# riusricardo/midnight-bls12-381-cuda

Measured on AMD Instinct MI355X. Metric: G1 MSM/sec at 2^20 points + Fr NTT/sec at 2^22 (bit-exact vs BLST), higher is better.
Workload: dtype u32-limb Montgomery (Fq 381-bit / Fr 255-bit integer); 1 GPU; G1 MSM 2^20 points per GPU, production path (ICICLE entry, Montgomery scalars + bases in HBM, (x,y,1) result on device); N>1: sharded, RCCL all-gather of partial sums; msm_points_per_gpu=1048576, ntt_size=4194304, parallelism=msm-shard1

## Files before the change

include/bls12_381_mi355x.h:

```cpp
#ifndef BLS12_381_MI355X_H
#define BLS12_381_MI355X_H

#include <stddef.h>
#include <stdint.h>
#include <stdbool.h>

#ifdef __cplusplus
extern "C" {
#endif

typedef enum {
    MBLS_SUCCESS = 0,
    MBLS_INVALID_DEVICE = 1,
    MBLS_OUT_OF_MEMORY = 2,
    MBLS_INVALID_POINTER = 3,
    MBLS_ALLOCATION_FAILED = 4,
    MBLS_DEALLOCATION_FAILED = 5,
    MBLS_COPY_FAILED = 6,
    MBLS_SYNCHRONIZATION_FAILED = 7,
    MBLS_STREAM_CREATION_FAILED = 8,
    MBLS_STREAM_DESTRUCTION_FAILED = 9,
    MBLS_API_NOT_IMPLEMENTED = 10,
    MBLS_INVALID_ARGUMENT = 11,
    MBLS_BACKEND_LOAD_FAILED = 12,
// ... 176 lines not shown
eIcicleError bls12_381_g1_scalar_mul_glv(const mbls_g1_affine_t* bases, const mbls_fr_t* scalars, int size,
                                         const VecOpsConfig* config, mbls_g1_projective_t* output);
eIcicleError bls12_381_g2_scalar_mul(const mbls_g2_affine_t* bases, const mbls_fr_t* scalars, int size,
                                     const VecOpsConfig* config, mbls_g2_projective_t* output);
eIcicleError mbls_g1_scalar_mul(const mbls_g1_affine_t* bases, const mbls_fr_t* scalars, int size,
                                bool scalars_montgomery, const VecOpsConfig* config, mbls_g1_projective_t* output);
eIcicleError mbls_g2_scalar_mul(const mbls_g2_affine_t* bases, const mbls_fr_t* scalars, int size,
                                bool scalars_montgomery, const VecOpsConfig* config, mbls_g2_projective_t* output);

eIcicleError mbls_g1_ecntt(const mbls_g1_affine_t* input, int size, NTTDir dir, const NTTConfig* config,
                           mbls_g1_affine_t* output);

typedef enum {
    MBLS_POINT_OK = 0,
    MBLS_POINT_IDENTITY = 1,
    MBLS_POINT_NONCANONICAL = 2,
    MBLS_POINT_OFF_CURVE = 3,
    MBLS_POINT_OFF_SUBGROUP = 4
} mbls_point_status;

eIcicleError mbls_g1_check_points(const mbls_g1_affine_t* points, int size, bool points_montgomery,
                                  const VecOpsConfig* config, uint8_t* status, uint64_t* n_invalid);
eIcicleError mbls_g2_check_points(const mbls_g2_affine_t* points, int size, bool points_montgomery,
                                  const VecOpsConfig* config, uint8_t* status, uint64_t* n_invalid);

typedef enum {
    MBLS_DECODE_OK = 0,
    MBLS_DECODE_IDENTITY = 1,
    MBLS_DECODE_NONCANONICAL = 2,
    MBLS_DECODE_NO_POINT = 3,
    MBLS_DECODE_BAD_FLAGS = 5
} mbls_decode_status;

eIcicleError mbls_g1_decompress(const uint8_t* bytes, int size, bool points_montgomery, const VecOpsConfig* config,
                                mbls_g1_affine_t* points, uint8_t* status, uint64_t* n_invalid);
eIcicleError mbls_g2_decompress(const uint8_t* bytes, int size, bool points_montgomery, const VecOpsConfig* config,
                                mbls_g2_affine_t* points, uint8_t* status, uint64_t* n_invalid);
eIcicleError mbls_g1_compress(const mbls_g1_affine_t* points, int size, bool points_montgomery,
                              const VecOpsConfig* config, uint8_t* bytes);
eIcicleError mbls_g2_compress(const mbls_g2_affine_t* points, int size, bool points_montgomery,
                              const VecOpsConfig* config, uint8_t* bytes);

const char* mbls_version(void);
const char* mbls_error_string(eIcicleError e);
eIcicleError mbls_gen_scalars(mbls_fr_t* out_device, uint64_t seed, size_t n, bool montgomery, void* stream);
eIcicleError mbls_gen_g1_bases(mbls_g1_affine_t* out_device, uint64_t seed, size_t n, void* stream);
eIcicleError mbls_gen_g2_bases(mbls_g2_affine_t* out_device, uint64_t seed, size_t n, void* stream);
eIcicleError mbls_gen_scalars_range(mbls_fr_t* out_device, uint64_t seed, size_t start, size_t n, bool montgomery,
                                    void* stream);
eIcicleError mbls_gen_g1_bases_range(mbls_g1_affine_t* out_device, uint64_t seed, size_t start, size_t n, void* stream);
eIcicleError mbls_gen_g2_bases_range(mbls_g2_affine_t* out_device, uint64_t seed, size_t start, size_t n, void* stream);
eIcicleError mbls_g1_msm_jacobian(const mbls_fr_t* scalars, const mbls_g1_affine_t* bases, int msm_size,
                                  const MSMConfig* config, mbls_g1_projective_t* results);
eIcicleError mbls_g2_msm_jacobian(const mbls_fr_t* scalars, const mbls_g2_affine_t* bases, int msm_size,
                                  const MSMConfig* config, mbls_g2_projective_t* results);
eIcicleError mbls_g1_sum_jacobian(const mbls_g1_projective_t* points_device, int count,
                                  mbls_g1_projective_t* result_device, void* stream);
eIcicleError mbls_g2_sum_jacobian(const mbls_g2_projective_t* points_device, int count,
                                  mbls_g2_projective_t* result_device, void* stream);
eIcicleError mbls_g1_jacobian_to_icicle(mbls_g1_projective_t* points_device, int count, void* stream);
eIcicleError mbls_g2_jacobian_to_icicle(mbls_g2_projective_t* points_device, int count, void* stream);

eIcicleError mbls_release_stream(void* stream);
eIcicleError mbls_release_scratch(void);
void mbls_scratch_stats(uint64_t* mallocs, uint64_t* frees, uint64_t* bytes, int* contexts);

eIcicleError mbls_g1_msm_multi_device(const mbls_fr_t* scalars, const mbls_g1_affine_t* const* bases_per_dev,
                                      const int* devs, int ndev, int msm_size, const MSMConfig* config,
                                      mbls_g1_projective_t* result);
eIcicleError mbls_g2_msm_multi_device(const mbls_fr_t* scalars, const mbls_g2_affine_t* const* bases_per_dev,
                                      const int* devs, int ndev, int msm_size, const MSMConfig* config,
                                      mbls_g2_projective_t* result);

eIcicleError bls12_381_vector_sum(const mbls_fr_t* a, size_t size, const VecOpsConfig* config, mbls_fr_t* output);

eIcicleError mbls_msm_plan(int group, int msm_size, const MSMConfig* config, int32_t* out);

eIcicleError mbls_msm_reduce_plan(int group, int msm_size, const MSMConfig* config, int32_t* out, int capacity,
                                  int32_t* count);

eIcicleError mbls_msm_front_probe(int group, const mbls_fr_t* scalars, const void* bases, int msm_size,
                                  const MSMConfig* config, int64_t* info, void* const* tables);

void mbls_profile_enable(int on);
void mbls_profile_reset(void);
int mbls_profile_read(const char** names, double* total_ms, long* counts, int max);

eIcicleError mbls_msm_accumulate_event(void* stream, void* event);
eIcicleError mbls_msm_accumulate_event_drop(void* event);

eIcicleError mbls_msm_precompute_strict(int on);

#ifdef __cplusplus
}
#endif
#endif
```

midnight-bls12-381-cuda_amd/bls12_381_amd.py:

```python
from __future__ import annotations

import ctypes
import os

import numpy as np

HERE = os.path.dirname(os.path.abspath(__file__))
LIB_PATH = os.environ.get("MBLS_LIB") or os.path.join(HERE, "lib", "libbls12_381_mi355x.so")

ERRORS = ["SUCCESS", "INVALID_DEVICE", "OUT_OF_MEMORY", "INVALID_POINTER", "ALLOCATION_FAILED",
          "DEALLOCATION_FAILED", "COPY_FAILED", "SYNCHRONIZATION_FAILED", "STREAM_CREATION_FAILED",
          "STREAM_DESTRUCTION_FAILED", "API_NOT_IMPLEMENTED", "INVALID_ARGUMENT", "BACKEND_LOAD_FAILED",
          "LICENSE_CHECK_ERROR", "UNKNOWN_ERROR"]
SUCCESS, INVALID_POINTER, API_NOT_IMPLEMENTED, INVALID_ARGUMENT = 0, 3, 10, 11


class IcicleError(RuntimeError):
    def __init__(self, code, what):
        name = ERRORS[code] if 0 <= code < len(ERRORS) else str(code)
        super().__init__(f"{what} failed: {name} ({code})")
        self.code = code


class MSMConfig(ctypes.Structure):
    _fields_ = [("stream", ctypes.c_void_p), ("precompute_factor", ctypes.c_int), ("c", ctypes.c_int),
                ("bitsize", ctypes.c_int), ("batch_size", ctypes.c_int),
                ("are_points_shared_in_batch", ctypes.c_bool), ("are_scalars_on_device", ctypes.c_bool),
                ("are_scalars_montgomery_form", ctypes.c_bool), ("are_points_on_device", ctypes.c_bool),
                ("are_points_montgomery_form", ctypes.c_bool), ("are_results_on_device", ctypes.c_bool),
                ("is_async", ctypes.c_bool), ("ext", ctypes.c_void_p)]


class FrC(ctypes.Structure):
    _fields_ = [("limbs", ctypes.c_uint64 * 4)]


class NTTConfig(ctypes.Structure):
    _fields_ = [("stream", ctypes.c_void_p), ("coset_gen", FrC), ("batch_size", ctypes.c_int),
                ("columns_batch", ctypes.c_bool), ("ordering", ctypes.c_int),
                ("are_inputs_on_device", ctypes.c_bool), ("are_outputs_on_device", ctypes.c_bool),
                ("is_async", ctypes.c_bool), ("ext", ctypes.c_void_p)]


class NTTInitDomainConfig(ctypes.Structure):
    _fields_ = [("stream", ctypes.c_void_p), ("is_async", ctypes.c_bool), ("ext", ctypes.c_void_p)]


class VecOpsConfig(ctypes.Structure):
    _fields_ = [("stream", ctypes.c_void_p), ("is_a_on_device", ctypes.c_bool), ("is_b_on_device", ctypes.c_bool),
                ("is_result_on_device", ctypes.c_bool), ("is_async", ctypes.c_bool), ("batch_size", ctypes.c_int),
                ("columns_batch", ctypes.c_bool), ("ext", ctypes.c_void_p)]


EXPORTED = [
    "mbls_default_msm_config", "mbls_default_ntt_config", "mbls_default_vec_ops_config",
    "bls12_381_g1_msm_cuda", "bls12_381_g2_msm_cuda", "bls12_381_icicle_g1_msm", "bls12_381_icicle_g2_msm",
    "bls12_381_icicle_g1_msm_precompute_bases", "bls12_381_icicle_g2_msm_precompute_bases",
    "bls12_381_ntt_init_domain_cuda", "bls12_381_ntt_release_domain_cuda", "bls12_381_ntt_cuda",
    "bls12_381_coset_ntt_cuda", "bls12_381_field_ntt_cuda", "bls12_381_field_ntt_init_domain_cuda",
    "bls12_381_field_ntt_release_domain_cuda", "bls12_381_ntt_get_rou_from_domain",
    "bls12_381_vector_add", "bls12_381_vector_sub", "bls12_381_vector_mul", "bls12_381_scalar_mul_vec",
    "bls12_381_scalar_add_vec", "vec_add_cuda", "vec_sub_cuda", "vec_mul_cuda", "scalar_mul_vec_cuda",
    "scalar_add_vec_cuda", "vec_sum_cuda", "bls12_381_batch_inv_cuda",
    "mbls_version", "mbls_error_string", "mbls_gen_scalars", "mbls_gen_g1_bases", "mbls_gen_g2_bases",
    "mbls_gen_scalars_range", "mbls_gen_g1_bases_range", "mbls_gen_g2_bases_range",
    "mbls_g1_msm_jacobian", "mbls_g2_msm_jacobian",
    "mbls_g1_sum_jacobian", "mbls_g2_sum_jacobian", "mbls_g1_jacobian_to_icicle", "mbls_g2_jacobian_to_icicle",
    "mbls_profile_enable", "mbls_profile_reset", "mbls_profile_read",
    "mbls_release_stream", "mbls_release_scratch", "mbls_scratch_stats",
    "mbls_g1_msm_multi_device", "mbls_g2_msm_multi_device", "bls12_381_vector_sum",
    "bls12_381_g1_affine_to_projective", "bls12_381_g1_projective_to_affine", "bls12_381_g2_projective_to_affine",
    "mbls_msm_plan", "mbls_msm_reduce_plan", "mbls_msm_front_probe", "mbls_msm_accumulate_event", "mbls_msm_accumulate_event_drop", "mbls_msm_precompute_strict",
    "bls12_381_g1_scalar_mul", "bls12_381_g1_scalar_mul_glv", "bls12_381_g2_scalar_mul",
    "mbls_g1_scalar_mul", "mbls_g2_scalar_mul", "mbls_g1_ecntt",
    "mbls_g1_check_points", "mbls_g2_check_points",
    "mbls_g1_decompress", "mbls_g2_decompress", "mbls_g1_compress", "mbls_g2_compress",
    "mbls_fr_prefix_product", "mbls_fr_poly_divide_linear", "mbls_fr_scan_geometry",
    "mbls_fr_eval_program", "mbls_fr_expr_check",
    "mbls_fr_sort", "mbls_fr_lookup_permute", "mbls_fr_sort_plan",
    "mbls_fr_coeff_to_extended", "mbls_fr_extended_to_coeff", "mbls_fr_domain_plan",
    "mbls_fr_lookup_multiplicities", "mbls_fr_prefix_sum", "mbls_fr_logup_sum",
]

_LIB = None


def lib():
    global _LIB
    if _LIB is not None:
        return _LIB
    if not os.path.exists(LIB_PATH):
        raise RuntimeError(f"HIP library not built: {LIB_PATH} (run __graft_entry__.build())")
    L = ctypes.CDLL(LIB_PATH)
    P, E = ctypes.c_void_p, ctypes.c_int
    sz, i32, u64, b = ctypes.c_size_t, ctypes.c_int, ctypes.c_uint64, ctypes.c_bool
    sig = {
        "bls12_381_g1_msm_cuda": [P, P, i32, P, P], "bls12_381_g2_msm_cuda": [P, P, i32, P, P],
        "bls12_381_icicle_g1_msm": [P, P, i32, P, P], "bls12_381_icicle_g2_msm": [P, P, i32, P, P],
        "bls12_381_icicle_g1_msm_precompute_bases": [P, i32, P, P],
        "bls12_381_icicle_g2_msm_precompute_bases": [P, i32, P, P],
        "bls12_381_ntt_init_domain_cuda": [P, P], "bls12_381_ntt_release_domain_cuda": [],
        "bls12_381_ntt_cuda": [P, i32, i32, P, P], "bls12_381_coset_ntt_cuda": [P, i32, i32, P, P, P],
        "bls12_381_field_ntt_cuda": [P, i32, i32, P, P], "bls12_381_field_ntt_init_domain_cuda": [P, P],
        "bls12_381_field_ntt_release_domain_cuda": [], "bls12_381_ntt_get_rou_from_domain": [u64, P],
        "bls12_381_vector_add": [P, P, sz, P, P], "bls12_381_vector_sub": [P, P, sz, P, P],
        "bls12_381_vector_mul": [P, P, sz, P, P], "bls12_381_scalar_mul_vec": [P, P, sz, P, P],
        "bls12_381_scalar_add_vec": [P, P, sz, P, P],
        "vec_add_cuda": [P, P, P, i32, P], "vec_sub_cuda": [P, P, P, i32, P], "vec_mul_cuda": [P, P, P, i32, P],
        "scalar_mul_vec_cuda": [P, P, P, i32, P], "scalar_add_vec_cuda": [P, P, P, i32, P],
        "vec_sum_cuda": [P, P, i32, P], "bls12_381_batch_inv_cuda": [P, P, i32, P],
        "mbls_gen_scalars": [P, u64, sz, b, P], "mbls_gen_g1_bases": [P, u64, sz, P],
        "mbls_gen_g2_bases": [P, u64, sz, P], "mbls_g1_sum_jacobian": [P, i32, P, P],
        "mbls_gen_scalars_range": [P, u64, sz, sz, b, P], "mbls_gen_g1_bases_range": [P, u64, sz, sz, P],
        "mbls_gen_g2_bases_range": [P, u64, sz, sz, P],
        "mbls_g1_msm_jacobian": [P, P, i32, P, P], "mbls_g2_msm_jacobian": [P, P, i32, P, P],
        "mbls_g2_sum_jacobian": [P, i32, P, P], "mbls_g1_jacobian_to_icicle": [P, i32, P],
        "mbls_g2_jacobian_to_icicle": [P, i32, P],
        "mbls_release_stream": [P], "mbls_release_scratch": [],
        "mbls_g1_msm_multi_device": [P, P, P, i32, i32, P, P], "mbls_g2_msm_multi_device": [P, P, P, i32, i32, P, P],
        "bls12_381_vector_sum": [P, sz, P, P],
        "bls12_381_g1_affine_to_projective": [P, i32, P, P], "bls12_381_g1_projective_to_affine": [P, i32, P, P],
        "bls12_381_g2_projective_to_affine": [P, i32, P, P],
        "mbls_msm_plan": [i32, i32, P, P], "mbls_msm_reduce_plan": [i32, i32, P, P, i32, P],
        "mbls_msm_front_probe": [i32, P, P, i32, P, P, P],
        "mbls_msm_accumulate_event": [P, P], "mbls_msm_accumulate_event_drop": [P],
        "mbls_msm_precompute_strict": [i32],
        "bls12_381_g1_scalar_mul": [P, P, i32, P, P], "bls12_381_g1_scalar_mul_glv": [P, P, i32, P, P],
        "bls12_381_g2_scalar_mul": [P, P, i32, P, P],
        "mbls_g1_scalar_mul": [P, P, i32, b, P, P], "mbls_g2_scalar_mul": [P, P, i32, b, P, P],
        "mbls_g1_ecntt": [P, i32, i32, P, P],
        "mbls_g1_check_points": [P, i32, b, P, P, P], "mbls_g2_check_points": [P, i32, b, P, P, P],
        "mbls_g1_decompress": [P, i32, b, P, P, P, P], "mbls_g2_decompress": [P, i32, b, P, P, P, P],
        "mbls_g1_compress": [P, i32, b, P, P], "mbls_g2_compress": [P, i32, b, P, P],
        "mbls_fr_prefix_product": [P, P, sz, P, b, P, P, P], "mbls_fr_poly_divide_linear": [P, sz, P, P, P, P],
        "mbls_fr_scan_geometry": [sz, P],
        "mbls_fr_eval_program": [P, i32, sz, sz, P, i32, P, i32, i32, P, P],
        "mbls_fr_expr_check": [P, i32, i32, i32, i32, P],
        "mbls_fr_sort": [P, sz, b, P, P, P], "mbls_fr_lookup_permute": [P, P, sz, b, P, P, P, P],
        "mbls_fr_sort_plan": [sz, i32, P],
        "mbls_fr_coeff_to_extended": [P, i32, i32, P, P, P],
        "mbls_fr_extended_to_coeff": [P, i32, i32, P, P, i32, P, P], "mbls_fr_domain_plan": [i32, i32, P],
        "mbls_fr_lookup_multiplicities": [P, i32, P, sz, b, b, P, P, P],
        "mbls_fr_prefix_sum": [P, sz, P, b, P, P, P], "mbls_fr_logup_sum": [P, i32, P, P, sz, P, P, P, P, P],
    }
    for name, args in sig.items():
        f = getattr(L, name)
        f.argtypes = args
        f.restype = E
    L.mbls_version.restype = ctypes.c_char_p
    L.mbls_error_string.restype = ctypes.c_char_p
    L.mbls_error_string.argtypes = [E]
    L.mbls_default_msm_config.restype = MSMConfig
    L.mbls_default_ntt_config.restype = NTTConfig
    L.mbls_default_vec_ops_config.restype = VecOpsConfig
    L.mbls_profile_enable.argtypes = [ctypes.c_int]
    L.mbls_profile_enable.restype = None
    L.mbls_profile_reset.argtypes = []
    L.mbls_profile_reset.restype = None
    L.mbls_profile_read.argtypes = [ctypes.POINTER(ctypes.c_char_p), ctypes.POINTER(ctypes.c_double),
                                    ctypes.POINTER(ctypes.c_long), ctypes.c_int]
    L.mbls_profile_read.restype = ctypes.c_int
    L.mbls_scratch_stats.argtypes = [ctypes.POINTER(ctypes.c_uint64)] * 3 + [ctypes.POINTER(ctypes.c_int)]
    L.mbls_scratch_stats.restype = None
    _LIB = L
    return L


def profile(enable=True):
    lib().mbls_profile_enable(1 if enable else 0)
    lib().mbls_profile_reset()


def profile_read():
    n = 64
    names = (ctypes.c_char_p * n)()
    ms = (ctypes.c_double * n)()
    cnt = (ctypes.c_long * n)()
    k = lib().mbls_profile_read(names, ms, cnt, n)
    return {names[i].decode(): (ms[i], cnt[i]) for i in range(min(k, n))}


def check(code, what):
    if code != SUCCESS:
        raise IcicleError(code, what)


def _p(x):
    if x is None:
        return None
    if isinstance(x, np.ndarray):
        assert x.flags["C_CONTIGUOUS"]
        return ctypes.c_void_p(x.ctypes.data)
    return ctypes.c_void_p(x.data_ptr())


def _is_dev(x):
    return x is not None and not isinstance(x, np.ndarray) and bool(getattr(x, "is_cuda", True))


def _stream_handle(stream):
    if stream is None:
        return None
    if isinstance(stream, int):
        return ctypes.c_void_p(stream)
    return ctypes.c_void_p(stream.cuda_stream)


def msm_config(**kw):
    c = lib().mbls_default_msm_config()
    for k, v in kw.items():
        if k == "stream":
            c.stream = _stream_handle(v)
        else:
            setattr(c, k, v)
    return c


PLAN_FIELDS = ("c", "W", "Wg", "F", "sF", "split", "prepared", "bstride", "buckets", "levels")


def msm_plan(group, n, **cfg):
    out = (ctypes.c_int32 * len(PLAN_FIELDS))()
    c = msm_config(**cfg)
    check(lib().mbls_msm_plan(1 if group == "g1" else 2, n, ctypes.byref(c), out), "msm_plan")
    return dict(zip(PLAN_FIELDS, list(out)))


REDUCE_KERNELS = ("chain", "tree4", "r28x", "tree8", "r28px")
REDUCE_MODES = ("lane", "row", "wave")
REDUCE_LEVEL_FIELDS = ("kernel", "launch", "mode", "seg_log", "m_in", "raw_in", "raw_out")


def msm_reduce_plan(group, n, **cfg):
    out = (ctypes.c_int32 * 128)()
    cnt = ctypes.c_int32(0)
    c = msm_config(**cfg)
    check(lib().mbls_msm_reduce_plan(1 if group == "g1" else 2, n, ctypes.byref(c), out, len(out), ctypes.byref(cnt)),
          "msm_reduce_plan")
    levels = []
    for k in range(2, cnt.value, len(REDUCE_LEVEL_FIELDS)):
        lv = dict(zip(REDUCE_LEVEL_FIELDS, out[k:k + len(REDUCE_LEVEL_FIELDS)]))
        lv["kernel"], lv["mode"] = REDUCE_KERNELS[lv["kernel"]], REDUCE_MODES[lv["mode"]]
        levels.append(lv)
    return dict(bucket_raw=out[0], level_bytes=out[1], levels=levels)


FRONT_PLAN_FIELDS = ("c", "W", "Wg", "F", "sF", "split", "prepared", "bstride", "B", "TB", "chunk", "pts",
                     "contributions", "partition_sort", "fused_chunk_counts")
FRONT_TABLES = ("sorted", "offsets", "nchunks", "chunk_off", "owner", "first", "perm", "binbase", "H_bucket",
                "H_first", "H_nslices", "H_done", "H_owner", "H_gdone")
FRONT_FILL = 0xA5A5A5A5


def msm_front_plan(group, n, **cfg):
    c = msm_config(**cfg)
    info = (ctypes.c_int64 * (len(FRONT_PLAN_FIELDS) + len(FRONT_TABLES)))()
    check(lib().mbls_msm_front_probe(1 if group == "g1" else 2, None, None, n, ctypes.byref(c), info, None),
          "msm_front_probe")
    k = len(FRONT_PLAN_FIELDS)
    return dict(plan=dict(zip(FRONT_PLAN_FIELDS, list(info)[:k])), words=dict(zip(FRONT_TABLES, list(info)[k:])))


def msm_front_tables(group, scalars, bases=None, *, n=None, c=0, bitsize=0, precompute_factor=1, scalars_mont=False,
                     points_mont=True, stream=None):
    if n is None:
        n = scalars.shape[0]
    cfg = msm_config(c=c, bitsize=bitsize, precompute_factor=precompute_factor,
                     are_scalars_on_device=_is_dev(scalars), are_scalars_montgomery_form=scalars_mont,
                     are_points_on_device=_is_dev(bases), are_points_montgomery_form=points_mont, stream=stream)
    g = 1 if group == "g1" else 2
    info = (ctypes.c_int64 * (len(FRONT_PLAN_FIELDS) + len(FRONT_TABLES)))()
    check(lib().mbls_msm_front_probe(g, None, None, n, ctypes.byref(cfg), info, None), "msm_front_probe")
    words = list(info)[len(FRONT_PLAN_FIELDS):]
    tabs = [np.zeros(w, dtype=np.uint32) for w in words]
    ptrs = (ctypes.c_void_p * len(tabs))(*[t.ctypes.data for t in tabs])
    check(lib().mbls_msm_front_probe(g, _p(scalars), _p(bases), n, ctypes.byref(cfg), info, ptrs), "msm_front_probe")
    assert list(info)[len(FRONT_PLAN_FIELDS):] == words
    return dict(plan=dict(zip(FRONT_PLAN_FIELDS, list(info))), tables=dict(zip(FRONT_TABLES, tabs)))


def ntt_config(**kw):
    c = lib().mbls_default_ntt_config()
    for k, v in kw.items():
        if k == "stream":
            c.stream = _stream_handle(v)
        elif k == "coset_gen":
            for i in range(4):
                c.coset_gen.limbs[i] = int(v[i])
        else:
            setattr(c, k, v)
    return c


def vec_config(**kw):
    c = lib().mbls_default_vec_ops_config()
    for k, v in kw.items():
        if k == "stream":
            c.stream = _stream_handle(v)
        else:
            setattr(c, k, v)
    return c


_VEC = {"add": "bls12_381_vector_add", "sub": "bls12_381_vector_sub", "mul": "bls12_381_vector_mul",
        "scalar_mul": "bls12_381_scalar_mul_vec", "scalar_add": "bls12_381_scalar_add_vec"}


def vec_op(op, a, b, out=None, stream=None, is_async=False, batch=1, columns_batch=False):
    total = b.shape[0]
    if out is None:
        out = np.zeros((total, 4), dtype=np.uint64)
    cfg = vec_config(is_a_on_device=_is_dev(a), is_b_on_device=_is_dev(b), is_result_on_device=_is_dev(out),
                     is_async=is_async, stream=stream, batch_size=batch, columns_batch=columns_batch)
    check(getattr(lib(), _VEC[op])(_p(a), _p(b), total // batch, ctypes.byref(cfg), _p(out)), _VEC[op])
    return out


_CONV = {("g1", "to_projective"): ("bls12_381_g1_affine_to_projective", 18),
         ("g1", "to_affine"): ("bls12_381_g1_projective_to_affine", 12),
         ("g2", "to_affine"): ("bls12_381_g2_projective_to_affine", 24)}


def convert_points(group, direction, pts, out=None, stream=None, is_async=False):
    name, words = _CONV[(group, direction)]
    n = pts.shape[0]
    if out is None:
        out = np.zeros((n, words), dtype=np.uint64)
    cfg = vec_config(is_a_on_device=_is_dev(pts), is_result_on_device=_is_dev(out), stream=stream, is_async=is_async)
    check(getattr(lib(), name)(_p(pts), n, ctypes.byref(cfg), _p(out)), name)
    return out


def scalar_mul(group, bases, scalars, *, scalars_mont=False, out=None, stream=None, is_async=False):
    n = bases.shape[0]
    assert scalars.shape[0] == n
    if out is None:
        out = np.zeros((n, 18 if group == "g1" else 36), dtype=np.uint64)
    cfg = vec_config(is_a_on_device=_is_dev(bases), is_b_on_device=_is_dev(scalars), is_result_on_device=_is_dev(out),
                     stream=stream, is_async=is_async)
    name = "mbls_g1_scalar_mul" if group == "g1" else "mbls_g2_scalar_mul"
    check(getattr(lib(), name)(_p(bases), _p(scalars), n, bool(scalars_mont), ctypes.byref(cfg), _p(out)), name)
    return out


POINT_OK, POINT_IDENTITY, POINT_NONCANONICAL, POINT_OFF_CURVE, POINT_OFF_SUBGROUP = range(5)


def check_points(group, pts, *, points_mont=True, out=None, count=True, stream=None, is_async=False):
    n = pts.shape[0]
    if out is None:
        out = np.zeros(n, dtype=np.uint8)
    elif out is False:
        out = None
    cnt = ctypes.c_uint64(0) if count else None
    cfg = vec_config(is_a_on_device=_is_dev(pts), is_result_on_device=_is_dev(out), stream=stream, is_async=is_async)
    name = "mbls_g1_check_points" if group == "g1" else "mbls_g2_check_points"
    check(getattr(lib(), name)(_p(pts), n, bool(points_mont), ctypes.byref(cfg), _p(out),
                               ctypes.byref(cnt) if count else None), name)
    return out, (int(cnt.value) if count else None)


DECODE_OK, DECODE_IDENTITY, DECODE_NONCANONICAL, DECODE_NO_POINT, DECODE_BAD_FLAGS = 0, 1, 2, 3, 5

# ... 475 lines not shown
```

midnight-bls12-381-cuda_amd/csrc/mbls_wavepoint.hpp:

```cpp
#pragma once
#include <type_traits>

#include "mbls_curve.hpp"
#include "mbls_rowfield.hpp"

namespace mbls {
namespace wave {

MBLS_DEV uint32_t row() { return (__lane_id() >> 4) & 3u; }

template <int K>
MBLS_DEV void mul4(RFq* r, const RFq* a, const RFq* b) {
    static_assert(K >= 1 && K <= 4, "one product per row");
    uint32_t A = a[0].v, B = b[0].v;
#pragma unroll
    for (int k = 1; k < K; ++k) {
        const uint64_t rowk = 0xffffull << (16 * k);
        A = rowop::pick(rowk, A, a[k].v);
        B = rowop::pick(rowk, B, b[k].v);
    }
    const RFq p = RFq{A} * RFq{B};
    const int l16 = (int)rowdpp::lane16();
#pragma unroll
    for (int k = 0; k < K; ++k) r[k].v = (uint32_t)__shfl((int)p.v, l16 + 16 * k, 64);
// ... 97 lines not shown
    }
    muln<N>(P, A, B);
#pragma unroll
    for (int k = 0; k < KS; ++k) {
        rs[k].c0 = P[2 * k];
        rs[k].c1 = dbl(P[2 * k + 1]);
    }
#pragma unroll
    for (int k = 0; k < KM; ++k) {
        const int o = 2 * KS + 3 * k;
        rm[k].c0 = P[o] - P[o + 1];
        rm[k].c1 = (P[o + 2] - P[o]) - P[o + 1];
    }
}

template <class RF>
MBLS_DEV Jacobian<RF> jdbl(const Jacobian<RF>& p) {
    if (p.is_inf()) return p;
    Jacobian<RF> r;
    if constexpr (std::is_same<RF, RFq>::value) {
        RF m1[3];
        mul<3>(m1, {p.x, p.y, x2_in(p.y)}, {add_in(x2_in(p.x), p.x), p.y, p.z});
        const RF E = m1[0], B = m1[1];
        RF m2[4];
        mul<4>(m2, {E, x4_in(p.x), x8_in(p.x), x8_in(B)}, {E, B, B, B});
        const RF D = m2[1];
        r.x = m2[0] - m2[2];
        RF m3[1];
        mul<1>(m3, {E}, {D - r.x});
        r.y = m3[0] - m2[3];
        r.z = m1[2];
    } else {
        RF s1[2], m1[1];
        sqr_mul<2, 1>(s1, m1, {p.x, p.y}, {p.y}, {p.z});
        const RF A = s1[0], B = s1[1];
        const RF E = dbl(A) + A;
        RF s2[2], m2[1];
        sqr_mul<2, 1>(s2, m2, {B, E}, {p.x}, {B});
        const RF C = s2[0];
        const RF D = dbl(dbl(m2[0]));
        r.x = s2[1] - dbl(D);
        RF m3[1];
        mul<1>(m3, {E}, {D - r.x});
        r.y = m3[0] - dbl(dbl(dbl(C)));
        r.z = dbl(m1[0]);
    }
    return r;
}

template <class RF>
MBLS_DEV Jacobian<RF> jadd(const Jacobian<RF>& p, const Jacobian<RF>& q) {
    if (p.is_inf()) return q;
    if (q.is_inf()) return p;
    RF s1[2], m1[1];
    sqr_mul<2, 1>(s1, m1, {p.z, q.z}, {p.z}, {q.z});
    const RF Z1Z1 = s1[0], Z2Z2 = s1[1];
    RF m2[4];
    mul<4>(m2, {p.x, q.x, q.z, p.z}, {Z2Z2, Z1Z1, Z2Z2, Z1Z1});
    const RF U1 = m2[0], U2 = m2[1];
    const RF H = U2 - U1;
    const RF H2 = x2_in(H);
    RF s3[1], m3[2];
    sqr_mul<1, 2>(s3, m3, {H2}, {p.y, q.y}, {m2[2], m2[3]});
    const RF S1 = m3[0];
    const RF R = m3[1] - S1;
    if (H.is_zero()) {
        if (R.is_zero()) return jdbl(p);
        return Jacobian<RF>::inf();
    }
    const RF I = s3[0];
    const RF R2 = x2_in(R);
    RF s4[1], m4[3];
    sqr_mul<1, 3>(s4, m4, {R2}, {H, U1, x2_in(m1[0])}, {I, I, H});
    const RF J = m4[0], V = m4[1];
    Jacobian<RF> r;
    r.x = s4[0] - J - dbl(V);
    r.z = m4[2];
    RF m5[2];
    mul<2>(m5, {R2, x2_in(S1)}, {V - r.x, J});
    r.y = m5[0] - m5[1];
    return r;
}

MBLS_DEV bool leader_row() { return row() == 0; }

}
}
```

midnight-bls12-381-cuda_amd/csrc/msm_core.hpp:

```cpp
#pragma once
#include <hip/hip_runtime.h>
#include <stdio.h>
#include <string.h>

#include <algorithm>
#include <type_traits>
#include <vector>

#include "mbls_common.hpp"
#include "mbls_curve.hpp"
#include "mbls_fq28.hpp"
#include "mbls_fq2_28.hpp"
#include "mbls_rowfield.hpp"
#include "mbls_wavepoint.hpp"

namespace mbls {

static constexpr uint32_t INVALID_KEY = 0xffffffffu;

#ifndef MBLS_SETPRIO
#define MBLS_SETPRIO 3
#endif
#define MBLS_TAIL_PRIO() __builtin_amdgcn_s_setprio(MBLS_SETPRIO)
#ifndef MBLS_LIGHT_PRIO
// ... 934 lines not shown
    }
    MBLS_DEV static RFq get1(const uint32_t* s) {
        const uint32_t j = rowdpp::lane16();
        return {j < 12 ? s[j] : 0u};
    }
    MBLS_DEV static void put1(uint32_t* s, const RFq2& a) {
        put1(s, a.c0);
        put1(s + 12, a.c1);
    }
    MBLS_DEV static void get1(const uint32_t* s, RFq2& a) {
        a.c0 = get1(s);
        a.c1 = get1(s + 12);
    }
    MBLS_DEV static void get1(const uint32_t* s, RFq& a) { a = get1(s); }
    MBLS_DEV static void put(uint32_t* s, const J& p) {
        put1(s, p.x);
        put1(s + 12 * FQS, p.y);
        put1(s + 24 * FQS, p.z);
    }
    MBLS_DEV static J get(const uint32_t* s) {
        J p;
        get1(s, p.x);
        get1(s + 12 * FQS, p.y);
        get1(s + 24 * FQS, p.z);
        return p;
    }
};

template <class F>
__global__ __launch_bounds__(256) void k_reduce_tree4(const uint8_t* __restrict__ V, const uint8_t* __restrict__ U,
                                                      uint32_t m_in, uint8_t* __restrict__ Vout,
                                                      uint8_t* __restrict__ Uout) {
    MBLS_TAIL_PRIO();
    using IO = RedIO<F, MODE_WAVE>;
    using J = RJac<F>;
    using T = TreeLds<F>;
    __shared__ uint32_t slot[8][T::WORDS];
    const uint32_t m_out = (m_in + 3) >> 2;
    const uint32_t seg = blockIdx.x;
    const uint32_t w = seg / m_out, q = seg % m_out;
    const uint32_t k0 = q << 2, cnt = min(4u, m_in - k0);
    const size_t base = (size_t)w * m_in + k0;
    const int wv = (int)__builtin_amdgcn_readfirstlane(threadIdx.x >> 6);
    auto ldV = [&](uint32_t t) { return t < cnt ? IO::ld(V, base + t) : J::inf(); };
    auto ldU = [&](uint32_t t) { return (U && t < cnt) ? IO::ld(U, base + t) : J::inf(); };
    J r = J::inf();
    for (int step = 0; step < 3; ++step) {
        const bool active = step < 2 || wv == 0;
        J x = J::inf(), y = J::inf();
        if (step == 0) {
            x = wv == 0 ? ldV(2) : wv == 1 ? ldU(0) : wv == 2 ? ldU(2) : ldV(0);
            y = wv == 0 ? ldV(3) : wv == 1 ? ldU(1) : wv == 2 ? ldU(3) : ldV(1);
        } else if (step == 1) {
            x = wv == 2 ? T::get(slot[1]) : wv == 3 ? T::get(slot[3]) : T::get(slot[0]);
            y = wv == 0 ? ldV(3) : wv == 1 ? ldV(1) : wv == 2 ? T::get(slot[2]) : T::get(slot[0]);
        } else if (active) {
            x = T::get(slot[5]);
            y = r;
        }
        if (active) r = IO::add(x, y);
        if (step < 2) {
            T::put(slot[4 * step + wv], r);
            __syncthreads();
        }
    }
    if (wv == 0) {
        IO::st(Uout, seg, IO::add(r, T::get(slot[6])));
    } else if (wv == 3 && Vout) {
        for (int k = 0; k < 2; ++k) r = IO::dbl(r);
        IO::st(Vout, seg, r);
    }
}

template <class F, int MODE>
MBLS_DEV auto final_fold(const uint8_t* __restrict__ windows, int Wg, int c) {
    using IO = RedIO<F, MODE>;
    auto acc = IO::ld(windows, Wg - 1);
    for (int w = Wg - 2; w >= 0; --w) {
        for (int k = 0; k < c; ++k) acc = IO::dbl(acc);
        acc = IO::add(acc, IO::ld(windows, w));
    }
    return acc;
}
template <class F>
__global__ void k_final(const uint8_t* __restrict__ windows, int Wg, int c, uint8_t* __restrict__ result) {
    MBLS_TAIL_PRIO();
    using IO = RedIO<F, MODE_WAVE>;
    if (IO::id() != 0) return;
    IO::st(result, 0, final_fold<F, MODE_WAVE>(windows, Wg, c));
}

template <class F>
__global__ void k_store_inf(uint8_t* result, int count) {
    int i = blockIdx.x * blockDim.x + threadIdx.x;
    if (i < count) store_jac<F>(result, i, Jacobian<F>::inf());
}

MBLS_DEV Fq to_mont_f(const Fq& a) { return to_mont(a); }
MBLS_DEV Fq2 to_mont_f(const Fq2& a) { return {to_mont(a.c0), to_mont(a.c1)}; }
MBLS_DEV Fq from_mont_f(const Fq& a) { return from_mont(a); }
MBLS_DEV Fq2 from_mont_f(const Fq2& a) { return {from_mont(a.c0), from_mont(a.c1)}; }
template <class F>
MBLS_DEV F one_std();
template <>
MBLS_DEV Fq one_std<Fq>() {
    Fq r = Fq::zero();
    r.v[0] = 1;
    return r;
}
template <>
MBLS_DEV Fq2 one_std<Fq2>() {
    Fq2 r = Fq2::zero();
    r.c0.v[0] = 1;
    return r;
}

template <class F>
__global__ void k_points_to_mont(uint8_t* pts, size_t n) {
    size_t i = blockIdx.x * (size_t)blockDim.x + threadIdx.x;
    if (i >= n) return;
    Affine<F> p = load_affine<F>(pts, i);
    p.x = to_mont_f(p.x);
    p.y = to_mont_f(p.y);
    store_affine<F>(pts, i, p);
}

MBLS_DEV RFq from_mont_f(const RFq& a) { return from_mont(a); }
MBLS_DEV RFq2 from_mont_f(const RFq2& a) { return {from_mont(a.c0), from_mont(a.c1)}; }
template <>
MBLS_DEV RFq one_std<RFq>() {
    return {rowdpp::lane16() == 0 ? 1u : 0u};
}
template <>
MBLS_DEV RFq2 one_std<RFq2>() {
    return {one_std<RFq>(), RFq::zero()};
}

template <class F>
MBLS_DEV void icicle_point(const Jacobian<F>& p, uint8_t* out, size_t i) {
    Jacobian<F> o;
    if (p.is_inf()) {
        o.x = F::zero();
        o.y = one_std<F>();
        o.z = F::zero();
    } else {
        Affine<F> a = jac_to_affine(p);
        o.x = from_mont_f(a.x);
        o.y = from_mont_f(a.y);
        o.z = one_std<F>();
    }
    store_jac<F>(out, i, o);
}

template <class F>
MBLS_DEV void icicle_point_quad(const Jacobian<F>& p, uint8_t* out, size_t i) {
    Jacobian<F> o;
    if (p.is_inf()) {
        o.x = F::zero();
        o.y = one_std<F>();
        o.z = F::zero();
    } else {
        const F zi = inv_quad(p.z);
        const F zi2 = sqr(zi);
        o.x = from_mont_f(p.x * zi2);
        o.y = from_mont_f(p.y * zi2 * zi);
        o.z = one_std<F>();
    }
    if ((__lane_id() & 3u) == 0) store_jac<F>(out, i, o);
}

template <class F>
__global__ __launch_bounds__(64) void k_jac_to_icicle(const uint8_t* in, uint8_t* out, int count) {
    const int i = (int)(blockIdx.x * blockDim.x + threadIdx.x);
    if (i >= count) return;
    icicle_point<F>(load_jac<F>(in, i), out, i);
}

MBLS_DEV Fq row_to_lane(const RFq& a) {
    Fq r;
#pragma unroll
    for (int i = 0; i < 12; ++i) r.v[i] = (uint32_t)__shfl((int)a.v, i, 64);
    return r;
}
MBLS_DEV Fq2 row_to_lane(const RFq2& a) { return {row_to_lane(a.c0), row_to_lane(a.c1)}; }

template <class F>
__global__ __launch_bounds__(64) void k_final_icicle(const uint8_t* __restrict__ windows, int Wg, int c,
                                                     uint8_t* __restrict__ out) {
    MBLS_TAIL_PRIO();
    const RJac<F> acc = final_fold<F, MODE_WAVE>(windows, Wg, c);
    Jacobian<F> p;
    p.x = row_to_lane(acc.x);
    p.y = row_to_lane(acc.y);
    p.z = row_to_lane(acc.z);
    if (threadIdx.x < 4) icicle_point_quad<F>(p, out, 0);
}

template <class F>
__global__ void k_sum_jac(const uint8_t* pts, int count, uint8_t* out) {
    using IO = RedIO<F, MODE_WAVE>;
    if (IO::id() != 0) return;
    auto acc = RJac<F>::inf();
    for (int i = 0; i < count; ++i) acc = IO::add(acc, IO::ld(pts, i));
    IO::st(out, 0, acc);
}

template <class F>
MBLS_DEV Affine<F> generator();
template <>
MBLS_DEV Affine<Fq> generator<Fq>() { return g1_generator(); }
template <>
MBLS_DEV Affine<Fq2> generator<Fq2>() { return g2_generator(); }

MBLS_DEV uint64_t splitmix64(uint64_t x) {
    x += 0x9e3779b97f4a7c15ULL;
    x = (x ^ (x >> 30)) * 0xbf58476d1ce4e5b9ULL;
    x = (x ^ (x >> 27)) * 0x94d049bb133111ebULL;
    return x ^ (x >> 31);
}

MBLS_DEV Fr gen_scalar(uint64_t seed, uint64_t i) {
    uint64_t base = splitmix64(seed) ^ (i * 0xd1342543de82ef95ULL);
    Fr s;
#pragma unroll
    for (int j = 0; j < 4; ++j) {
        uint64_t l = splitmix64(base + (uint64_t)j * 0x632be59bd9b4e019ULL);
        if (j == 3) l &= 0x7fffffffffffffffULL;
        s.v[2 * j] = (uint32_t)l;
        s.v[2 * j + 1] = (uint32_t)(l >> 32);
    }
    reduce_once(s);
    return s;
}

template <class F>
__global__ void k_gen_bases(uint8_t* out, uint64_t seed, size_t start, size_t n) {
    size_t i = blockIdx.x * (size_t)blockDim.x + threadIdx.x;
    if (i >= n) return;
    Fr k = gen_scalar(seed, start + i);
    Jacobian<F> g = Jacobian<F>::from_affine(generator<F>());
    store_affine<F>(out, i, jac_to_affine(jac_mul_u32(g, k.v)));
}

template <class F>
__global__ __launch_bounds__(128) void k_precompute(const uint8_t* in, uint8_t* out, size_t n, int factor, int shift) {
    size_t i = blockIdx.x * (size_t)blockDim.x + threadIdx.x;
    if (i >= n) return;
    Affine<F> a = load_affine<F>(in, i);
    store_affine<F>(out, i * factor, a);
    Jacobian<F> p = Jacobian<F>::from_affine(a);
    for (int f = 1; f < factor; ++f) {
        for (int k = 0; k < shift; ++k) p = jac_dbl(p);
        store_affine<F>(out, i * factor + f, jac_to_affine(p));
    }
}


inline bool msm_image_table(const MsmPlan& P) { return P.split > 1 && !P.prepared; }
template <class F>
inline size_t msm_scratch(const MsmPlan& P, uint8_t* base, MsmScratch& S) {
    constexpr size_t jac = PointSize<F>::JAC, aff = PointSize<F>::AFF;
    size_t used = 0;
    auto take = [&](auto*& p, size_t bytes) {
        p = base ? reinterpret_cast<std::remove_reference_t<decltype(p)>>(base + used) : nullptr;
        used += align_up(bytes);
    };
    const bool psort = partition_sort(P);
    const PartSortSizes ps = psort ? part_sort_sizes(P) : PartSortSizes();
    const size_t NC = P.contributions;
    const uint32_t max_chunks = (uint32_t)(NC / P.chunk + P.TB + 1);
    take(S.keys, 4 * (psort ? 0 : NC));
    take(S.vals, 4 * (psort ? 0 : NC));
    take(S.ranks, 4 * (psort ? 0 : NC));
    take(S.dsrc, digits_src_bytes((uint32_t)(P.split > 1 ? P.pts / P.split : P.pts / P.F), P.split));
    take(S.sorted, 4 * NC);
    const size_t tb_words = (size_t)P.TB + 4;
    take(S.counts, 4 * tb_words);
    take(S.offsets, 4 * tb_words);
// ... 462 lines not shown
```

midnight-bls12-381-cuda_amd/csrc/msm_g1.hip:

```cpp
#include "msm_core.hpp"

using namespace mbls;
using G = Fq;

extern "C" {

eIcicleError bls12_381_g1_msm_cuda(const mbls_fr_t* scalars, const mbls_g1_affine_t* bases, int msm_size,
                                   const MSMConfig* config, mbls_g1_projective_t* result) {
    return msm_call<G>(scalars, bases, msm_size, config, result, MSM_RAW);
}
eIcicleError bls12_381_icicle_g1_msm(const mbls_fr_t* scalars, const mbls_g1_affine_t* bases, int msm_size,
                                     const MSMConfig* config, mbls_g1_projective_t* results) {
    return msm_call<G>(scalars, bases, msm_size, config, results, MSM_ICICLE);
}
eIcicleError bls12_381_icicle_g1_msm_precompute_bases(const mbls_g1_affine_t* input_bases, int bases_size,
                                                      const MSMConfig* config, mbls_g1_affine_t* output_bases) {
    return precompute_call<G>(input_bases, bases_size, config, output_bases);
}
eIcicleError mbls_gen_g1_bases_range(mbls_g1_affine_t* out_device, uint64_t seed, size_t start, size_t n, void* stream) {
    if (!out_device) return MBLS_INVALID_POINTER;
    if (n == 0) return MBLS_SUCCESS;
    hipLaunchKernelGGL(k_gen_bases<G>, dim3((unsigned)((n + 127) / 128)), dim3(128), 0, (hipStream_t)stream,
                       (uint8_t*)out_device, seed, start, n);
    MBLS_TRY(hipGetLastError());
    return MBLS_SUCCESS;
}
eIcicleError mbls_gen_g1_bases(mbls_g1_affine_t* out_device, uint64_t seed, size_t n, void* stream) {
    return mbls_gen_g1_bases_range(out_device, seed, 0, n, stream);
}
eIcicleError mbls_g1_msm_jacobian(const mbls_fr_t* scalars, const mbls_g1_affine_t* bases, int msm_size, const MSMConfig* config,
                                   mbls_g1_projective_t* results) {
    return msm_call<G>(scalars, bases, msm_size, config, results, MSM_JACOBIAN);
}
eIcicleError mbls_g1_sum_jacobian(const mbls_g1_projective_t* pts, int count, mbls_g1_projective_t* result,
                                  void* stream) {
    if (!pts || !result || count < 0) return MBLS_INVALID_ARGUMENT;
    hipLaunchKernelGGL(k_sum_jac<G>, dim3(1), dim3(64), 0, (hipStream_t)stream, (const uint8_t*)pts, count,
                       (uint8_t*)result);
    MBLS_TRY(hipGetLastError());
    return MBLS_SUCCESS;
}
eIcicleError mbls_g1_jacobian_to_icicle(mbls_g1_projective_t* pts, int count, void* stream) {
    if (!pts || count < 0) return MBLS_INVALID_ARGUMENT;
    if (count == 0) return MBLS_SUCCESS;
    hipLaunchKernelGGL(k_jac_to_icicle<G>, dim3((count + 63) / 64), dim3(64), 0, (hipStream_t)stream, (const uint8_t*)pts, (uint8_t*)pts,
                       count);
    MBLS_TRY(hipGetLastError());
    return MBLS_SUCCESS;
}

eIcicleError mbls_g1_msm_multi_device(const mbls_fr_t* scalars, const mbls_g1_affine_t* const* bases_per_dev, const int* devs,
                                      int ndev, int msm_size, const MSMConfig* config, mbls_g1_projective_t* result) {
    return msm_multi_device<G>(scalars, reinterpret_cast<const void* const*>(bases_per_dev), devs, ndev, msm_size, config,
                               result);
}

}
```

Measured before the change: 288.2 MSM/s.

## Switch G1 final window fold to projective coordinates with complete formulas

For G1, the final window fold (Horner over window sums with c doublings per window) now runs in a scaled homogeneous projective representation with 4-way batched Montgomery multiplies, instead of the Jacobian fold. Window sums are converted Jacobian-to-projective in groups of four, and the result is converted back or normalized to affine for the ICICLE output. The aim is fewer field multiplies and more multiply parallelism in this single-wave serial tail kernel. It also adds a probe entry point for testing the fold on its own. The tail is small relative to the whole MSM, and the new formulas must stay bit-exact.

```diff
diff --git a/include/bls12_381_mi355x.h b/include/bls12_381_mi355x.h
--- a/include/bls12_381_mi355x.h
+++ b/include/bls12_381_mi355x.h
@@ -282,6 +282,9 @@
 eIcicleError mbls_msm_front_probe(int group, const mbls_fr_t* scalars, const void* bases, int msm_size,
                                   const MSMConfig* config, int64_t* info, void* const* tables);
 
+eIcicleError mbls_g1_fold_probe(const mbls_g1_projective_t* windows, int Wg, int c, int jacobian,
+                                mbls_g1_projective_t* out, void* stream);
+
 void mbls_profile_enable(int on);
 void mbls_profile_reset(void);
 int mbls_profile_read(const char** names, double* total_ms, long* counts, int max);
diff --git a/midnight-bls12-381-cuda_amd/bls12_381_amd.py b/midnight-bls12-381-cuda_amd/bls12_381_amd.py
--- a/midnight-bls12-381-cuda_amd/bls12_381_amd.py
+++ b/midnight-bls12-381-cuda_amd/bls12_381_amd.py
@@ -70,7 +70,7 @@
     "mbls_release_stream", "mbls_release_scratch", "mbls_scratch_stats",
     "mbls_g1_msm_multi_device", "mbls_g2_msm_multi_device", "bls12_381_vector_sum",
     "bls12_381_g1_affine_to_projective", "bls12_381_g1_projective_to_affine", "bls12_381_g2_projective_to_affine",
-    "mbls_msm_plan", "mbls_msm_reduce_plan", "mbls_msm_front_probe", "mbls_msm_accumulate_event", "mbls_msm_accumulate_event_drop", "mbls_msm_precompute_strict",
+    "mbls_msm_plan", "mbls_msm_reduce_plan", "mbls_msm_front_probe", "mbls_g1_fold_probe", "mbls_msm_accumulate_event", "mbls_msm_accumulate_event_drop", "mbls_msm_precompute_strict",
     "bls12_381_g1_scalar_mul", "bls12_381_g1_scalar_mul_glv", "bls12_381_g2_scalar_mul",
     "mbls_g1_scalar_mul", "mbls_g2_scalar_mul", "mbls_g1_ecntt",
     "mbls_g1_check_points", "mbls_g2_check_points",
@@ -123,6 +123,7 @@
         "bls12_381_g2_projective_to_affine": [P, i32, P, P],
         "mbls_msm_plan": [i32, i32, P, P], "mbls_msm_reduce_plan": [i32, i32, P, P, i32, P],
         "mbls_msm_front_probe": [i32, P, P, i32, P, P, P],
+        "mbls_g1_fold_probe": [P, i32, i32, i32, P, P],
         "mbls_msm_accumulate_event": [P, P], "mbls_msm_accumulate_event_drop": [P],
         "mbls_msm_precompute_strict": [i32],
         "bls12_381_g1_scalar_mul": [P, P, i32, P, P], "bls12_381_g1_scalar_mul_glv": [P, P, i32, P, P],
@@ -279,6 +280,15 @@
     return dict(plan=dict(zip(FRONT_PLAN_FIELDS, list(info))), tables=dict(zip(FRONT_TABLES, tabs)))
 
 
+def g1_fold_probe(windows, c, *, jacobian=False, stream=None):
+    import torch
+    assert windows.is_cuda and windows.is_contiguous() and windows.shape[1] == 18
+    out = torch.zeros((1, 18), dtype=torch.int64, device=windows.device)
+    check(lib().mbls_g1_fold_probe(_p(windows), windows.shape[0], c, 1 if jacobian else 0, _p(out),
+                                   _stream_handle(stream)), "g1_fold_probe")
+    return out
+
+
 def ntt_config(**kw):
     c = lib().mbls_default_ntt_config()
     for k, v in kw.items():
diff --git a/midnight-bls12-381-cuda_amd/csrc/mbls_wavepoint.hpp b/midnight-bls12-381-cuda_amd/csrc/mbls_wavepoint.hpp
--- a/midnight-bls12-381-cuda_amd/csrc/mbls_wavepoint.hpp
+++ b/midnight-bls12-381-cuda_amd/csrc/mbls_wavepoint.hpp
@@ -203,6 +203,81 @@
     return r;
 }
 
+struct PFq {
+    RFq x, y, z;
+    MBLS_DEV static PFq inf() { return {RFq::zero(), RFq::one(), RFq::zero()}; }
+    MBLS_DEV bool is_inf() const { return z.is_zero(); }
+};
+struct PFqW {
+    RFq x, y, w;
+    MBLS_DEV bool is_inf() const { return w.is_zero(); }
+};
+
+MBLS_DEV RFq x3_in(const RFq& a) { return add_in(x2_in(a), a); }
+MBLS_DEV RFq x6_in(const RFq& a) { return x2_in(x3_in(a)); }
+MBLS_DEV RFq times6(const RFq& a) {
+    const RFq a2 = dbl(a);
+    return dbl(a2 + a);
+}
+MBLS_DEV PFqW to_w(const PFq& p) { return {p.x, p.y, times6(p.z)}; }
+MBLS_DEV PFq from_w(const PFqW& p) { return {times6(p.x), times6(p.y), p.w}; }
+
+MBLS_DEV PFqW pdbl(const PFqW& p) {
+    RFq m1[4];
+    mul<4>(m1, {p.y, x2_in(p.y), p.w, x2_in(p.x)}, {p.y, x4_in(p.w), p.w, x3_in(p.y)});
+    const RFq A = m1[0], C = m1[2];
+    const RFq d = A - C;
+    const RFq A3 = x3_in(A);
+    RFq m2[4];
+    mul<4>(m2, {d, A3, d, x8_in(A)}, {m1[3], m1[1], add_in(A3, C), C});
+    return {m2[0], m2[2] + m2[3], m2[1]};
+}
+
+MBLS_DEV PFqW padd(const PFqW& p, const PFq& q) {
+    const RFq x6 = x6_in(p.x), y6 = x6_in(p.y);
+    RFq m1[4];
+    mul<4>(m1, {x6, y6, p.w, x6_in(p.x + p.y)}, {q.x, q.y, q.z, q.x + q.y});
+    const RFq t0 = m1[0], t1 = m1[1], t2 = m1[2];
+    const RFq t3 = (m1[3] - t0) - t1;
+    const RFq u4 = dbl(dbl(t2));
+    const RFq u = dbl(u4) + u4;
+    const RFq m = t1 - u;
+    const RFq s = t1 + u;
+    const RFq T = dbl(t0) + t0;
+    RFq m2[4];
+    mul<4>(m2, {add_in(y6, p.w), add_in(x6, p.w), t3, x2_in(T)}, {q.y + q.z, q.x + q.z, m, x3_in(t3)});
+    const RFq t4 = (m2[0] - t1) - t2;
+    const RFq y = (m2[1] - t0) - t2;
+    const RFq v = dbl(y) + y;
+    RFq m3[4];
+    mul<4>(m3, {x4_in(t4), x4_in(v), m, x2_in(s)}, {v, T, s, x3_in(t4)});
+    return {m2[2] - m3[0], m3[2] + m3[1], m3[3] + m2[3]};
+}
+
+template <int K>
+MBLS_DEV void jac_to_proj(PFq (&r)[K], const Jacobian<RFq> (&j)[K]) {
+    RFq zz[K], A[2 * K], B[2 * K], P[2 * K];
+#pragma unroll
+    for (int k = 0; k < K; ++k) A[k] = j[k].z;
+    muln<K>(zz, A, A);
+#pragma unroll
+    for (int k = 0; k < K; ++k) {
+        A[2 * k] = j[k].x, B[2 * k] = j[k].z;
+        A[2 * k + 1] = zz[k], B[2 * k + 1] = j[k].z;
+    }
+    muln<2 * K>(P, A, B);
+#pragma unroll
+    for (int k = 0; k < K; ++k) r[k] = {P[2 * k], j[k].is_inf() ? RFq::one() : j[k].y, P[2 * k + 1]};
+}
+
+MBLS_DEV Jacobian<RFq> proj_to_jac(const PFq& p) {
+    RFq m1[2];
+    mul<2>(m1, {p.x, p.z}, {p.z, p.z});
+    RFq m2[1];
+    mul<1>(m2, {p.y}, {m1[1]});
+    return {m1[0], m2[0], p.z};
+}
+
 MBLS_DEV bool leader_row() { return row() == 0; }
 
 }
diff --git a/midnight-bls12-381-cuda_amd/csrc/msm_core.hpp b/midnight-bls12-381-cuda_amd/csrc/msm_core.hpp
--- a/midnight-bls12-381-cuda_amd/csrc/msm_core.hpp
+++ b/midnight-bls12-381-cuda_amd/csrc/msm_core.hpp
@@ -1040,12 +1040,42 @@
     }
     return acc;
 }
+MBLS_DEV void fold_step_proj(wave::PFqW& acc, const wave::PFq& g, int w, int Wg, int c) {
+    if (w == Wg - 1) {
+        acc = wave::to_w(g);
+    } else if (w >= 0) {
+        for (int i = 0; i < c; ++i) acc = wave::pdbl(acc);
+        acc = wave::padd(acc, g);
+    }
+}
+MBLS_DEV wave::PFq final_fold_proj(const uint8_t* __restrict__ windows, int Wg, int c) {
+    using IO = RedIO<Fq, MODE_WAVE>;
+    using J = RJac<Fq>;
+    wave::PFqW acc{RFq::zero(), RFq::one(), RFq::zero()};
+    for (int top = Wg - 1; top >= 0; top -= 4) {
+        const J j[4] = {IO::ld(windows, top), top >= 1 ? IO::ld(windows, top - 1) : J::inf(),
+                        top >= 2 ? IO::ld(windows, top - 2) : J::inf(), top >= 3 ? IO::ld(windows, top - 3) : J::inf()};
+        wave::PFq g[4];
+        wave::jac_to_proj<4>(g, j);
+        fold_step_proj(acc, g[0], top, Wg, c);
+        fold_step_proj(acc, g[1], top - 1, Wg, c);
+        fold_step_proj(acc, g[2], top - 2, Wg, c);
+        fold_step_proj(acc, g[3], top - 3, Wg, c);
+    }
+    return wave::from_w(acc);
+}
+
 template <class F>
 __global__ void k_final(const uint8_t* __restrict__ windows, int Wg, int c, uint8_t* __restrict__ result) {
     MBLS_TAIL_PRIO();
     using IO = RedIO<F, MODE_WAVE>;
     if (IO::id() != 0) return;
-    IO::st(result, 0, final_fold<F, MODE_WAVE>(windows, Wg, c));
+    if constexpr (std::is_same<F, Fq>::value) {
+        const wave::PFq acc = final_fold_proj(windows, Wg, c);
+        IO::st(result, 0, acc.is_inf() ? RJac<F>::inf() : wave::proj_to_jac(acc));
+    } else {
+        IO::st(result, 0, final_fold<F, MODE_WAVE>(windows, Wg, c));
+    }
 }
 
 template <class F>
@@ -1146,12 +1176,31 @@
 __global__ __launch_bounds__(64) void k_final_icicle(const uint8_t* __restrict__ windows, int Wg, int c,
                                                      uint8_t* __restrict__ out) {
     MBLS_TAIL_PRIO();
-    const RJac<F> acc = final_fold<F, MODE_WAVE>(windows, Wg, c);
-    Jacobian<F> p;
-    p.x = row_to_lane(acc.x);
-    p.y = row_to_lane(acc.y);
-    p.z = row_to_lane(acc.z);
-    if (threadIdx.x < 4) icicle_point_quad<F>(p, out, 0);
+    if constexpr (std::is_same<F, Fq>::value) {
+        const wave::PFq acc = final_fold_proj(windows, Wg, c);
+        const Fq X = row_to_lane(acc.x), Y = row_to_lane(acc.y), Z = row_to_lane(acc.z);
+        if (threadIdx.x < 4) {
+            Jacobian<Fq> o;
+            if (Z.is_zero()) {
+                o.x = Fq::zero();
+                o.y = one_std<Fq>();
+                o.z = Fq::zero();
+            } else {
+                const Fq zi = inv_quad(Z);
+                o.x = from_mont_f(X * zi);
+                o.y = from_mont_f(Y * zi);
+                o.z = one_std<Fq>();
+            }
+            if ((__lane_id() & 3u) == 0) store_jac<Fq>(out, 0, o);
+        }
+    } else {
+        const RJac<F> acc = final_fold<F, MODE_WAVE>(windows, Wg, c);
+        Jacobian<F> p;
+        p.x = row_to_lane(acc.x);
+        p.y = row_to_lane(acc.y);
+        p.z = row_to_lane(acc.z);
+        if (threadIdx.x < 4) icicle_point_quad<F>(p, out, 0);
+    }
 }
 
 template <class F>
diff --git a/midnight-bls12-381-cuda_amd/csrc/msm_g1.hip b/midnight-bls12-381-cuda_amd/csrc/msm_g1.hip
--- a/midnight-bls12-381-cuda_amd/csrc/msm_g1.hip
+++ b/midnight-bls12-381-cuda_amd/csrc/msm_g1.hip
@@ -49,6 +49,20 @@
     return MBLS_SUCCESS;
 }
 
+eIcicleError mbls_g1_fold_probe(const mbls_g1_projective_t* windows, int Wg, int c, int jacobian,
+                                mbls_g1_projective_t* out, void* stream) {
+    if (!windows || !out) return MBLS_INVALID_POINTER;
+    if (Wg < 1 || Wg > 256 || c < 1 || c > 32 || ((uintptr_t)windows | (uintptr_t)out) % 16) return MBLS_INVALID_ARGUMENT;
+    if (jacobian)
+        hipLaunchKernelGGL(k_final<G>, dim3(1), dim3(64), 0, (hipStream_t)stream, (const uint8_t*)windows, Wg, c,
+                           (uint8_t*)out);
+    else
+        hipLaunchKernelGGL(k_final_icicle<G>, dim3(1), dim3(64), 0, (hipStream_t)stream, (const uint8_t*)windows, Wg, c,
+                           (uint8_t*)out);
+    MBLS_TRY(hipGetLastError());
+    return MBLS_SUCCESS;
+}
+
 eIcicleError mbls_g1_msm_multi_device(const mbls_fr_t* scalars, const mbls_g1_affine_t* const* bases_per_dev, const int* devs,
                                       int ndev, int msm_size, const MSMConfig* config, mbls_g1_projective_t* result) {
     return msm_multi_device<G>(scalars, reinterpret_cast<const void* const*>(bases_per_dev), devs, ndev, msm_size, config,
```

Measured after the change: 284.4 MSM/s. 0.987x the previous value.
